# zhangganlin/GlORIE-SLAM

Hardware: AMD Instinct MI355X
Metric: DSPO BA-update iters/sec + rendered rays/sec, 640x480 Replica keyframe graph (higher is better)
Workload: dtype f16 corr/ConvGRU, f32 Jacobians, f64 solve; render: f32 (decoder matmuls as 3-term f16 splits, f32 accumulate); 1 GPU; G8: 8 keyframes, 36 edges, 60x80 (640x480/8), BA itrs=2, DSPO stages alternating, context part of the GRU gates (one map per source keyframe) re-evaluated for all keyframes every 12 steps; multiview_filter.thresh = 0.25 (reference ships 0.01, configs/mono_point_slam.yaml:75: with untrained weights 0.01 rejects > 80 % of every frame and no depth_scale step would reach stage 2); render: 524k-point c; edges_local=36, edges_total=36, hw=4800, keyframes=8, parallelism=single GPU

## Files before the change

### glorie_slam_amd/_lib.py

```python
import ctypes
import os
import threading

import torch

_PKG_DIR = os.path.dirname(os.path.abspath(__file__))
LIB_PATH = os.path.join(_PKG_DIR, "lib", "libglorie_hip.so")

GLORIE_F16, GLORIE_F32 = 0, 1
_STATUS = {0: "GLORIE_OK", -1: "GLORIE_EINVAL", -2: "GLORIE_EHIP", -3: "GLORIE_ENOMEM",
           -4: "GLORIE_EUNSUPPORTED"}

_c_int, _c_f, _vp, _sz = ctypes.c_int, ctypes.c_float, ctypes.c_void_p, ctypes.c_size_t

SIGNATURES = {
    "glorie_version": (ctypes.c_char_p, []),
    "glorie_last_hip_error": (_c_int, []),
    "glorie_ctx_create": (_c_int, [ctypes.POINTER(_vp), _sz]),
    "glorie_ctx_destroy": (_c_int, [_vp]),
    "glorie_ctx_reserve": (_c_int, [_vp, _sz]),
    "glorie_ctx_generation": (ctypes.c_ulonglong, [_vp]),
    "glorie_corr_index_fwd": (_c_int, [_vp, _vp, _vp] + [_c_int] * 7 + [_vp]),
    "glorie_corr_lookup_pyramid": (_c_int, [_vp, _c_int, _vp, _vp] + [_c_int] * 7 + [_vp]),
    "glorie_corr_otf": (_c_int, [_vp, _vp, _c_int, _vp, _vp, _vp, _vp] + [_c_int] * 4 + [_vp]),
    "glorie_corr_otf_encode": (_c_int, [_vp, _vp, _c_int, _vp, _vp, _vp, _vp] + [_c_int] * 4 + [_vp, _vp, _vp, _c_int, _vp]),
    "glorie_altcorr_fwd": (_c_int, [_vp] * 4 + [_c_int] * 8 + [_vp]),
    "glorie_bias_act": (_c_int, [_vp, _c_int, _vp, _vp, _c_int, ctypes.c_long, _c_int, _c_int, _vp]),
    "glorie_gru_glo_terms": (_c_int, [_vp, _c_int, _vp, _vp, _c_int, _vp, _vp, _c_int, _vp, _c_int, _vp, _c_int, _c_int, _vp]),
    "glorie_gru_gate_zr": (_c_int, [_vp, _c_int, _vp, _c_int, _vp, _c_int, _vp, _c_int, _vp, _c_int, _c_int, _c_int, _vp]),
    "glorie_gru_gate_q": (_c_int, [_vp, _c_int, _vp, _c_int, _vp, _c_int, _vp, _c_int, _vp, _c_int, _vp, _c_int, _c_int, _c_int, _vp]),
    "glorie_segment_mean": (_c_int, [_vp, _c_int, _vp, _c_int, _vp, _c_int, _vp, _c_int, _c_int, _c_int, _vp]),
    "glorie_conv3x3_small": (_c_int, [_vp, _c_int, _vp, _c_int, _vp, _vp, _c_int, _c_int, _c_int, ctypes.c_float, _vp, _vp, _c_int, _c_int, _c_int, _vp]),
    "glorie_gru_glo_from_tiles": (_c_int, [_vp, _vp, _vp, _c_int, _vp, _c_int, _c_int, _vp]),
    "glorie_update_bookkeeping": (_c_int, [_vp, _vp, _vp, ctypes.c_long, _vp, _vp, _vp, _vp, _c_int, _c_int, _c_f, _vp, _c_int,
                                           _vp]),
    "glorie_conv_igemm_heads": (_c_int, [_vp, _c_int, _c_int, _vp, _c_int, _c_int, _vp, _vp, _c_int, _c_int, _vp, _vp,
                                         _c_int, _c_int, _c_int, _c_int, _vp]),
    "glorie_conv_upsample": (_c_int, [_vp, _c_int, _c_int, _vp, _vp, _vp, _vp, _vp, _c_int, _c_int, _c_int, _c_int, _vp]),
    "glorie_conv_stencil": (_c_int, [_vp, _vp, _c_int, _c_int, _c_int, ctypes.c_float, _vp, _vp, _c_int, _c_int, _c_int, _vp]),
    "glorie_conv_igemm": (_c_int, [_vp, _c_int, _c_int, _vp, _c_int, _c_int, _vp, _c_int, _c_int, _c_int, _vp,
                                   _c_int, _c_int, _vp, _c_int, _vp, _c_int, _vp, _c_int, _vp, _c_int, _vp, _c_int, _vp,
                                   _c_int, _c_int, _c_int, _vp]),
    "glorie_flow_conv7": (_c_int, [_vp, _vp, _vp, _vp, _c_int, _c_int, _c_int, _c_int, _vp]),
    "glorie_motion": (_c_int, [_vp, _vp, _vp, _vp, _c_int, _c_int, _c_int, ctypes.c_float, _vp]),
    "glorie_motion_padded": (_c_int, [_vp, _vp, _vp, _vp, _c_int, _c_int, _c_int, ctypes.c_float, _vp]),
    "glorie_flow_pad": (_c_int, [_vp, _vp, _c_int, _c_int, _c_int, _vp]),
    "glorie_flow_conv7_padded": (_c_int, [_vp, _vp, _vp, _vp, _c_int, _c_int, _c_int, _c_int, _vp]),
    "glorie_flow_encoder": (_c_int, [_vp, _vp, _vp, _vp, _vp, _vp, _c_int, _c_int, _c_int, _c_int, _vp]),
    "glorie_publish_flag": (_c_int, [_vp, _vp, _vp, _vp]),
    "glorie_dspo_prepare": (_c_int, [_vp] * 4 + [_c_int] * 4 + [ctypes.c_float, _c_int, ctypes.c_float, _vp, _vp, _c_int] + [_vp] * 9),
    "glorie_corr_lookup_pyramid_tiled": (_c_int, [_vp, _c_int, _vp, _vp] + [_c_int] * 5 + [_vp]),
    "glorie_corr_build": (_c_int, [_vp] * 5 + [_c_int] * 5 + [_vp]),
    "glorie_corr_lookup_arena": (_c_int, [_vp, _c_int, _vp, _vp, _vp] + [_c_int] * 5 + [_vp]),
    "glorie_corr_lookup_tiled_cl": (_c_int, [_vp, _c_int, _vp, _vp, _c_int, _vp] + [_c_int] * 5 + [_vp]),
    "glorie_corr_dm_level_halfs": (ctypes.c_long, [_c_int, _c_int, _c_int]),
    "glorie_corr_dm_build": (_c_int, [_vp] * 5 + [_c_int] * 5 + [_vp]),
    "glorie_corr_dm_lookup": (_c_int, [_vp, _vp, _vp, _c_int, _c_int, _c_int, _c_int, _vp, _vp, _vp, _vp, _c_int, _vp]),
    "glorie_valid_depth_mask": (_c_int, [_vp] * 4 + [_c_int] * 4 + [ctypes.c_float, _c_int, _vp, _vp, _vp]),
    "glorie_reproject": (_c_int, [_vp] * 7 + [_c_int] * 3 + [_vp]),
    "glorie_reproject_motion": (_c_int, [_vp] * 9 + [_c_int] * 3 + [ctypes.c_float, _vp]),
    "glorie_frame_distance": (_c_int, [_vp] * 6 + [_c_int] * 3 + [_c_f, _vp]),
    "glorie_iproj": (_c_int, [_vp] * 4 + [_c_int] * 3 + [_vp]),
# ... 221 lines not shown
```

### glorie_slam_amd/csrc/gru.hip

```cpp
#include <hip/hip_runtime.h>
#include <stdint.h>
#include "common.hiph"

namespace glorie {

typedef __attribute__((ext_vector_type(8))) _Float16 h8;

__device__ __forceinline__ float sigmoidf_(float x) { return 1.0f / (1.0f + __expf(-x)); }
__device__ __forceinline__ float tanhf_(float x) {
  const float e = __expf(-2.0f * fabsf(x));
  const float t = (1.0f - e) / (1.0f + e);
  return copysignf(t, x);
}

enum { ACT_NONE = 0, ACT_RELU = 1, ACT_SIGMOID = 2, ACT_SOFTPLUS = 3 };

template <int C8T>
__global__ __launch_bounds__(256) void bias_act_kernel(const _Float16* __restrict__ x, int xs,
                                                       const float* __restrict__ bias,
                                                       _Float16* __restrict__ y, int ys, long P,
                                                       int C8R, int act) {
  const int C8 = C8T ? C8T : C8R;
  const long idx = (long)blockIdx.x * 256 + threadIdx.x;
  if (idx >= P * C8) return;
// ... 109 lines not shown
                                                         const _Float16* __restrict__ net, int ns,
                                                         _Float16* __restrict__ out, int os,
                                                         _Float16* __restrict__ out2, int os2, long P,
                                                         int HW) {
  const long idx = (long)blockIdx.x * 256 + threadIdx.x;
  if (idx >= P * 16) return;
  const long p = idx >> 4;
  const int c = (int)(idx & 15) * 8;
  const int n = (int)(p / HW);
  const h8 qv = *reinterpret_cast<const h8*>(qc + p * qs + c);
  const h8 zv = *reinterpret_cast<const h8*>(z + p * zs + c);
  const h8 nv = *reinterpret_cast<const h8*>(net + p * ns + c);
  h8 o;
#pragma unroll
  for (int k = 0; k < 8; ++k) {
    const float q = tanhf_((float)qv[k] + gq[(size_t)n * gs + c + k]);
    const float zz = (float)zv[k];
    o[k] = (_Float16)((1.0f - zz) * (float)nv[k] + zz * q);
  }
  *reinterpret_cast<h8*>(out + p * os + c) = o;
  if (out2) *reinterpret_cast<h8*>(out2 + p * os2 + c) = o;
}

__global__ __launch_bounds__(256) void segment_mean_kernel(const _Float16* __restrict__ x, int xs,
                                                           const float* __restrict__ bias, int relu,
                                                           const int64_t* __restrict__ ix, int N,
                                                           _Float16* __restrict__ out, int os, int HW) {
  __shared__ int elist[256];
  __shared__ int wcnt[4];
  const int tid = threadIdx.x, lane = tid & 63, wv = tid >> 6;
  const int idx = blockIdx.x * 256 + tid;
  const bool live = idx < HW * 16;
  const int p = idx >> 4, c = (idx & 15) * 8, g = blockIdx.y;
  float b[8] = {0, 0, 0, 0, 0, 0, 0, 0};
  if (bias) {
#pragma unroll
    for (int k = 0; k < 8; ++k) b[k] = bias[c + k];
  }
  float acc[8] = {0, 0, 0, 0, 0, 0, 0, 0};
  int cnt = 0;
  for (int base = 0; base < N; base += 256) {
    const int e = base + tid;
    const bool hit = e < N && ix[e] == g;
    const unsigned long long m = __ballot(hit);
    if (lane == 0) wcnt[wv] = __popcll(m);
    __syncthreads();
    int off = 0, total = 0;
#pragma unroll
    for (int q = 0; q < 4; ++q) {
      if (q < wv) off += wcnt[q];
      total += wcnt[q];
    }
    if (hit) elist[off + __popcll(m & ((1ull << lane) - 1ull))] = e;
    __syncthreads();
    if (live) {
      for (int q = 0; q < total; ++q) {
        const h8 v = *reinterpret_cast<const h8*>(x + ((long)elist[q] * HW + p) * xs + c);
#pragma unroll
        for (int k = 0; k < 8; ++k) {
          float f = (float)v[k] + b[k];
          if (relu) f = fmaxf(f, 0.0f);
          acc[k] += f;
        }
      }
    }
    cnt += total;
    __syncthreads();
  }
  if (!live) return;
  const float inv = 1.0f / (float)max(cnt, 1);
  h8 o;
#pragma unroll
  for (int k = 0; k < 8; ++k) o[k] = (_Float16)(acc[k] * inv);
  *reinterpret_cast<h8*>(out + ((long)g * HW + p) * os + c) = o;
}

typedef __attribute__((ext_vector_type(8))) _Float16 f16x8;
typedef __attribute__((ext_vector_type(4))) float f32x4;

template <int NT>
__global__ __launch_bounds__(256) void conv_taps_kernel(const _Float16* __restrict__ x, int xs,
                                                        const float* __restrict__ in_bias, int in_relu,
                                                        const f16x8* __restrict__ wp,
                                                        float* __restrict__ taps, int ncols, int tstride,
                                                        long P) {
  const int lane = threadIdx.x & 63, wv = threadIdx.x >> 6;
  const int col = lane & 15, kg = lane >> 4;
  const int grp = blockIdx.y;
  f16x8 bfrag[NT][4];
#pragma unroll
  for (int t = 0; t < NT; ++t)
#pragma unroll
    for (int kk = 0; kk < 4; ++kk) bfrag[t][kk] = wp[(((size_t)grp * NT + t) * 4 + kk) * 64 + lane];
  float ib[4][8];
#pragma unroll
  for (int kk = 0; kk < 4; ++kk)
#pragma unroll
// ... 17 lines not shown
        }
    }
#pragma unroll
    for (int t = 0; t < NT; ++t) {
      f32x4 acc = f32x4{0.f, 0.f, 0.f, 0.f};
#pragma unroll
      for (int kk = 0; kk < 4; ++kk)
        acc = __builtin_amdgcn_mfma_f32_16x16x32_f16(afrag[kk], bfrag[t][kk], acc, 0, 0, 0);
      const int n = t * 16 + col;
      if (n < ncols) {
#pragma unroll
        for (int r = 0; r < 4; ++r) {
          const long pr = p0 + kg * 4 + r;
          if (pr < P) taps[pr * tstride + grp * ncols + n] = acc[r];
        }
      }
    }
  }
}

__device__ __forceinline__ float softplusf_(float x) { return x > 20.0f ? x : log1pf(__expf(x)); }

template <bool PLANAR>
__global__ __launch_bounds__(256) void conv_stencil_kernel(const float* __restrict__ taps, int ncols,
                                                           int tstride, const float* __restrict__ bias,
                                                           int K, int groups, int act_packed, float scale,
                                                           float* __restrict__ out, long P, int H, int W,
                                                           float* __restrict__ out_last = nullptr) {
  const long idx = (long)blockIdx.x * 256 + threadIdx.x;
  if (idx >= P * K * groups) return;
  const int gk = PLANAR ? (int)(idx / P) : (int)(idx % (K * groups));
  const long p = PLANAR ? idx - (long)gk * P : idx / (K * groups);
  const int grp = gk / K, j = gk - grp * K;
  const int xw = (int)(p % W), yh = (int)((p / W) % H);
  float acc = bias ? bias[grp * K + j] : 0.0f;
#pragma unroll
  for (int d = 0; d < 9; ++d) {
    const int dy = d / 3 - 1, dx = d % 3 - 1;
    if ((unsigned)(yh + dy) < (unsigned)H && (unsigned)(xw + dx) < (unsigned)W)
      acc += PLANAR ? taps[(size_t)(grp * ncols + d * K + j) * P + (p + dy * W + dx)]
                    : taps[(p + dy * W + dx) * tstride + grp * ncols + d * K + j];
  }
  const int act = (act_packed >> (4 * grp)) & 15;
  if (act == ACT_RELU) acc = fmaxf(acc, 0.0f);
  else if (act == ACT_SIGMOID) acc = sigmoidf_(acc);
  else if (act == ACT_SOFTPLUS) acc = softplusf_(acc);
  if (out_last && grp == groups - 1) out_last[(size_t)p * K + j] = acc * scale;
  else out[((size_t)grp * P + p) * K + j] = acc * scale;
}

}

using namespace glorie;

extern "C" int glorie_bias_act(const void* x, int x_stride, const float* bias, void* y, int y_stride,
                               long P, int C, int act, void* stream) {
  if (P < 0 || C <= 0 || (C & 7) || (x_stride & 7) || (y_stride & 7)) return GLORIE_EINVAL;
  if (P == 0) return GLORIE_OK;
  if (!x || !y) return GLORIE_EINVAL;
  const long total = P * (C / 8);
  const dim3 grid((unsigned)((total + 255) / 256));
  auto launch = [&](auto kernel) {
    hipLaunchKernelGGL(kernel, grid, dim3(256), 0, (hipStream_t)stream,
                       reinterpret_cast<const _Float16*>(x), x_stride, bias,
                       reinterpret_cast<_Float16*>(y), y_stride, P, C / 8, act);
  };
  switch (C / 8) {
    case 8: launch(bias_act_kernel<8>); break;
    case 16: launch(bias_act_kernel<16>); break;
    case 48: launch(bias_act_kernel<48>); break;
    default: launch(bias_act_kernel<0>); break;
// ... 165 lines not shown
    hipLaunchKernelGGL(conv_taps_kernel<1>, dim3(gx, groups), dim3(256), 0, st,
                       reinterpret_cast<const _Float16*>(x), x_stride, in_bias, in_relu,
                       reinterpret_cast<const f16x8*>(w_packed), taps, ncols, tstride, P);
  else
    hipLaunchKernelGGL(conv_taps_kernel<2>, dim3(gx, groups), dim3(256), 0, st,
                       reinterpret_cast<const _Float16*>(x), x_stride, in_bias, in_relu,
                       reinterpret_cast<const f16x8*>(w_packed), taps, ncols, tstride, P);
  const long total = P * K * groups;
  hipLaunchKernelGGL(conv_stencil_kernel<false>, dim3((unsigned)((total + 255) / 256)), dim3(256), 0, st, taps,
                     ncols, tstride, out_bias, K, groups, act_packed, scale, out, P, H, W);
  return check_launch();
}

extern "C" int glorie_conv_stencil(const float* taps, const float* out_bias, int groups, int K, int act_packed,
                                   float scale, float* out, float* out_last, int N, int H, int W, void* stream) {
  if (N < 0 || H <= 0 || W <= 0 || groups < 1 || groups > 4 || K < 1 || K > 3) return GLORIE_EINVAL;
  if (N == 0) return GLORIE_OK;
  if (!taps || !out) return GLORIE_EINVAL;
  const long P = (long)N * H * W, total = P * K * groups;
  hipLaunchKernelGGL(conv_stencil_kernel<true>, dim3((unsigned)((total + 255) / 256)), dim3(256), 0, (hipStream_t)stream,
                     taps, 9 * K, 9 * K * groups, out_bias, K, groups, act_packed, scale, out, P, H, W, out_last);
  return check_launch();
}
```

### glorie_slam_amd/droid_net.py

```python
import os

import numpy as np
import torch
import torch.nn as nn
import torch.nn.functional as F

from . import droid_backends


def _conv(cin, cout, k):
    return nn.Conv2d(cin, cout, kernel_size=(k, k), padding=(k // 2, k // 2))


def cvx_upsample(data, mask):
    batch, ht, wd, dim = data.shape
    mask = mask.reshape(batch, 576, ht, wd)
    ix = torch.arange(batch, device=data.device)
    out = torch.empty(batch, 8 * ht, 8 * wd, dim, dtype=torch.float32, device=data.device)
    for c in range(dim):
        up = torch.empty(batch, 8 * ht, 8 * wd, dtype=torch.float32, device=data.device)
        droid_backends.cvx_upsample(data[..., c].float().contiguous(), ix, mask.contiguous(), up, softmax_f32=True)
        out[..., c] = up
    return out

# ... 193 lines not shown
    def __call__(self, net, inp, corr, flow=None, ii=None, jj=None, groups=None):
        self._sync()
        return self._net(self._cl(net), self._cl(inp), self._cl(corr), self._cl(flow), ii, jj, groups)


class FusedUpdate:

    def __init__(self, module, inplace=False):
        self.src = module
        self.inplace = inplace
        self.hoist_inp = True
        self._pre = None
        self.parallel = False
        self.glo_stream = True
        self._streams = None
        self._ver = None
        self._hx = None
        self._inp_key = None
        self._pre_kf, self._pre_map, self._ctx_key = None, None, None
        self._flow_pad = None
        self.fuse_glo = True
        self.fuse_heads = True
        self.fuse_flow = os.environ.get("GLORIE_FLOW_FUSED", "1") != "0"
        self.gate_events = None
        self.q_events = None
        self.heads_events = None
        self.corr_events = None

    def _sync(self):
        from . import update_ops as U
        ver = tuple(p._version for p in self.src.parameters())
        if self._ver == ver:
            return
        m = self.src
        f32 = lambda b: b.detach().float().contiguous()
        g = m.gru
        W = {}
        W["ce1_t"] = m.corr_encoder[0].weight.detach().view(128, -1).t().half().contiguous()
        W["ce1_b"] = f32(m.corr_encoder[0].bias)
        W["ce1_p"] = OtfCorrBlock.pack_encoder(m.corr_encoder[0].weight)
        W["ce1_cl"] = U.pack_corr_encoder(m.corr_encoder[0].weight)
        W["ce1_dm"] = U.pack_corr_encoder_dm(m.corr_encoder[0].weight)
        W["ce2"], W["ce2_b"] = U.pack_conv_igemm(m.corr_encoder[2].weight, pair=True), f32(m.corr_encoder[2].bias)
        W["fe1"], W["fe1_b"] = U.pack_flow_conv7(m.flow_encoder[0].weight), f32(m.flow_encoder[0].bias)
        W["fe2"], W["fe2_b"] = U.pack_conv_igemm(m.flow_encoder[2].weight, pair=True), f32(m.flow_encoder[2].bias)
        W["zr"] = U.pack_conv_igemm(torch.cat([g.convz.weight, g.convr.weight], 0), pair=True)
# ... 18 lines not shown
        W["up"], W["up_b"] = U.pack_conv_igemm(m.agg.upmask[0].weight), f32(m.agg.upmask[0].bias)
        W["up_cvx"], W["up_cvx_b"] = U.pack_upmask_conv(m.agg.upmask[0].weight, m.agg.upmask[0].bias)
        self.W = W
        self._ver = ver
        self._inp_key = None

    @torch.no_grad()
    def precompute_context(self):
        from . import update_ops as U
        hx = self._hx
        n, _, ht, wd = hx.shape
        if self._pre is None or self._pre.shape[0] != n or self._pre.shape[2:] != hx.shape[2:] \
                or self._pre.device != hx.device:
            self._pre = torch.empty((n, 384, ht, wd), dtype=torch.float16, device=hx.device,
                                    memory_format=torch.channels_last)
        U.conv_igemm(hx[:, 0:128], None, self.W["pre"], 9, 384, self._pre)
        return self._pre

    @staticmethod
    def _cl(t):
        b, n, c, h, w = t.shape
        return t.reshape(b * n, c, h, w).half().contiguous(memory_format=torch.channels_last)

    def _side_streams(self, dev):
        if self._streams is None or self._streams[0].device != dev:
            self._streams = (torch.cuda.Stream(dev), torch.cuda.Stream(dev))
        return self._streams

    @torch.no_grad()
    def precompute_shared_context(self, context):
        from . import update_ops as U
        table, frames, index = context
        g = int(frames.shape[0])
        ht, wd = table.shape[-2:]
        x = table[frames].half().contiguous(memory_format=torch.channels_last)
        if self._pre_kf is None or self._pre_kf.shape[0] < g or tuple(self._pre_kf.shape[2:]) != (ht, wd) \
                or self._pre_kf.device != x.device:
            self._pre_kf = torch.empty((max(g, 8), 384, ht, wd), dtype=torch.float16, device=x.device,
                                       memory_format=torch.channels_last)
        U.conv_igemm(x, None, self.W["pre"], 9, 384, self._pre_kf[:g])
        n = int(index.shape[0])
        if self._pre_map is None or self._pre_map.shape[0] < n or self._pre_map.device != x.device:
            self._pre_map = torch.zeros(max(n, 64), dtype=torch.int32, device=x.device)
        self._pre_map[:n].copy_(index)
        return self._pre_kf[:g], self._pre_map[:n]

    def _shared_context(self, context):
        table, frames, index = context
        key = (table.data_ptr(), table._version, frames.data_ptr(), frames._version, index.data_ptr(), index._version,
               int(frames.shape[0]), int(index.shape[0]), self._ver)
        if self._ctx_key != key:
            self.precompute_shared_context(context)
            self._ctx_key = key
            self._ctx_refs = (table, frames, index)
        return self._pre_kf[:int(frames.shape[0])], self._pre_map[:int(index.shape[0])]

    @torch.no_grad()
    def __call__(self, net, inp, corr, flow=None, ii=None, jj=None, groups=None, context=None, lazy_up=False,
                 weight_out=None):
        from . import update_ops as U
        self._sync()
        W = self.W
        batch, num, _, ht, wd = net.shape
        n, hw = batch * num, ht * wd
        dev = net.device
        cl_map = lambda c: torch.empty((n, c, ht, wd), dtype=torch.float16, device=dev,
                                       memory_format=torch.channels_last)
        if self._hx is None or tuple(self._hx.shape) != (n, 320, ht, wd) or self._hx.device != dev:
            self._hx = cl_map(320)
            self._inp_key = None
        hx = self._hx
        net0 = self._cl(net)
        main = torch.cuda.current_stream(dev)
        side = self._side_streams(dev) if self.parallel else ((main, self._side_streams(dev)[1]) if self.glo_stream
                                                              else (main, main))
        for st in side:
            if st is not main:
                st.wait_stream(main)
        with torch.cuda.stream(side[0]):
            if isinstance(flow, U.PaddedFlow):
                pf = flow
            else:
# ... 1 lines not shown
                    flow = torch.zeros(batch, num, 4, ht, wd, device=dev)
                fl = flow.reshape(n, 4, ht, wd).permute(0, 2, 3, 1).float().contiguous()
                if self._flow_pad is None or not self._flow_pad.fits(n, ht, wd, dev):
                    self._flow_pad = U.PaddedFlow(n, ht, wd, dev)
                pf = U.flow_pad(fl, self._flow_pad)
            if not (self.fuse_flow and U.flow_encoder(pf, W["fe1"], W["fe1_b"], W["fe2"], W["fe2_b"], hx[:, 256:320],
                                                      strict=False)):
                f1 = U.flow_conv7_padded(pf, W["fe1"], W["fe1_b"], cl_map(128))
                U.conv_igemm(f1, None, W["fe2"], 9, 64, hx[:, 256:320], terms=W["fe2_b"], act=U.ACT_RELU)
        shared = context is not None and self.hoist_inp
        with torch.cuda.stream(side[1]):
            if shared:
                pre_kf, pre_map = self._shared_context(context)
            elif self._inp_key is None or self._inp_key[0] is not inp or self._inp_key[1] != inp._version:
                U.bias_act(self._cl(inp), None, U.ACT_NONE, out=hx[:, 0:128])
                self._inp_key = (inp, inp._version)
                if self.hoist_inp:
                    self.precompute_context()
            if self.fuse_glo:
                g = U.gru_glo_terms_fused(net0, W["w"], W["w_b"], W["G"], W["G_b"])
            else:
                wn = U.conv_igemm(net0, None, W["w"], 1, 128, cl_map(128))
                g = U.gru_glo_terms(wn, W["w_b"], net0, W["G"], W["G_b"])
        if self.glo_stream and not self.parallel:
            main.wait_stream(side[1])
        if hasattr(corr, "encode_into"):
            c1 = cl_map(128)
            evc = self.corr_events
            if evc is not None:
                c0e, c1e = torch.cuda.Event(enable_timing=True), torch.cuda.Event(enable_timing=True)
                c0e.record()
            corr.encode_into(W, c1)
            if evc is not None:
                c1e.record()
                evc.append((c0e, c1e))
        else:
            if callable(corr):
                corr = corr()
            if corr.dim() == 4 and corr.shape[1] == 256 and corr.dtype == torch.float16:
                c1 = U.conv_igemm(corr, None, W["ce1_cl"], 1, 128, cl_map(128), terms=W["ce1_b"], act=U.ACT_RELU)
            else:
                c1 = torch.matmul(corr.reshape(n, -1, hw).half().transpose(1, 2), W["ce1_t"])
                c1 = c1.view(n, ht, wd, 128).permute(0, 3, 1, 2)
                U.bias_act(c1, W["ce1_b"], U.ACT_RELU)
        U.conv_igemm(c1, None, W["ce2"], 9, 128, hx[:, 128:256], terms=W["ce2_b"], act=U.ACT_RELU)
        for st in side:
            if st is not main:
                main.wait_stream(st)
        z, rnet = cl_map(128), cl_map(128)
        aliased = net0.data_ptr() == net.data_ptr() and net.dtype == torch.float16
        new = net0 if (self.inplace and aliased) else cl_map(128)
        if self.hoist_inp:
            dynx = hx[:, 128:320]
            pre, pmap = (pre_kf, pre_map) if shared else (self._pre, None)
            ev = self.gate_events
            if ev is not None:
                e0, e1 = torch.cuda.Event(enable_timing=True), torch.cuda.Event(enable_timing=True)
                e0.record()
            U.conv_igemm(net0, dynx, W["zr_dyn"], 9, 256, z, epilogue=U.EPI_GRU_ZR, terms=g[:, 0:256], net=net0,
                         out2=rnet, pre=pre[:, 0:256], pre_map=pmap)
            if ev is not None:
                e1.record()
                ev.append((e0, e1))
            evq = self.q_events
            if evq is not None:
                q0, q1 = torch.cuda.Event(enable_timing=True), torch.cuda.Event(enable_timing=True)
                q0.record()
            U.conv_igemm(rnet, dynx, W["q_dyn"], 9, 128, new, epilogue=U.EPI_GRU_Q, terms=g[:, 256:384], net=net0,
                         z=z, pre=pre[:, 256:384], pre_map=pmap)
            if evq is not None:
                q1.record()
                evq.append((q0, q1))
        else:
            U.conv_igemm(net0, hx, W["zr"], 9, 256, z, epilogue=U.EPI_GRU_ZR, terms=g[:, 0:256], net=net0, out2=rnet)
            U.conv_igemm(rnet, hx, W["q"], 9, 128, new, epilogue=U.EPI_GRU_Q, terms=g[:, 256:384], net=net0, z=z)
        net_out = new.view(batch, num, 128, ht, wd)
        if self.fuse_heads:
            agg_in = cl_map(128)
            evh = self.heads_events
            if evh is not None:
                h0, h1e = torch.cuda.Event(enable_timing=True), torch.cuda.Event(enable_timing=True)
                h0.record()
            rows = U.conv_igemm_heads(new, W["h1"], 9, 384, W["h1_b"], W["h2_taps"], 2, out=agg_in)
            if evh is not None:
                h1e.record()
                evh.append((h0, h1e))
            wo = weight_out if (weight_out is not None and weight_out.is_cuda and weight_out.dtype == torch.float32
                                and weight_out.is_contiguous() and weight_out.numel() == n * ht * wd * 2) else None
            dw = U.conv_stencil(rows, W["h2_b"], n, ht, wd, 2, 2, (U.ACT_NONE, U.ACT_SIGMOID), out_last=wo)
        else:
            h1 = U.conv_igemm(new, None, W["h1"], 9, 384, cl_map(384), terms=W["h1_b"], act=U.ACT_RELU)
            dw = U.conv3x3_small(h1, W["h2"], W["h2_b"], 2, (U.ACT_NONE, U.ACT_SIGMOID))
            agg_in = h1[:, 256:384]
        delta = dw[0].view(batch, num, ht, wd, 2)
        weight = dw[1].view(batch, num, ht, wd, 2) if (not self.fuse_heads or wo is None) else \
            weight_out.view(batch, num, ht, wd, 2)
        if ii is None:
            return net_out, delta, weight
        if groups is None:
            uniq, ix = torch.unique(ii.to(dev), sorted=True, return_inverse=True)
            ngroups = uniq.shape[0]
        else:
            ix, ngroups = groups
        agg = U.segment_mean(agg_in, ix.contiguous(), ngroups)
        a2 = torch.empty((ngroups, 128, ht, wd), dtype=torch.float16, device=dev,
                         memory_format=torch.channels_last)
        U.conv_igemm(agg, None, W["a2"], 9, 128, a2, terms=W["a2_b"], act=U.ACT_RELU)
        eta = U.conv3x3_small(a2, W["eta"], W["eta_b"], 1, (U.ACT_SOFTPLUS,), scale=0.01)
        if lazy_up:
            return net_out, delta, weight, eta.view(batch, ngroups, ht, wd), U.LazyUpmask(a2, W["up_cvx"], W["up_cvx_b"])
        up = torch.empty((ngroups, 576, ht, wd), dtype=torch.float16, device=dev,
                         memory_format=torch.channels_last)
        U.conv_igemm(a2, None, W["up"], 1, 576, up, terms=W["up_b"])
        return net_out, delta, weight, eta.view(batch, ngroups, ht, wd), up.view(batch, ngroups, 576, ht, wd)


class CorrBlock:

    def __init__(self, fmap1, fmap2, num_levels=4, radius=3, tiled=None):
        self.num_levels = num_levels
        self.radius = radius
        corr = CorrBlock.corr(fmap1, fmap2)
        batch, num, h1, w1, h2, w2 = corr.shape
        self.dims = (h1, w1, h2, w2)
        if tiled is None:
            tiled = corr.is_cuda and radius == 3 and (h1 * w1) % 8 == 0 and corr.dtype == torch.float16
        self.tiled = bool(tiled)
        corr = corr.reshape(batch * num * h1 * w1, 1, h2, w2)
        self.corr_pyramid = []
        for i in range(num_levels):
            if self.tiled:
# ... 298 lines not shown
```

### glorie_slam_amd/factor_graph.py

```python
import numpy as np
import os

import torch

from . import droid_backends
from .droid_net import ArenaLookup, CorrArena, CorrBlock, AltCorrBlock, FusedUpdate, FusedLookup, OtfCorrBlock


def coords_grid(ht, wd, device):
    y, x = torch.meshgrid(torch.arange(ht, device=device).float(),
                          torch.arange(wd, device=device).float(), indexing="ij")
    return torch.stack([x, y], dim=-1)


class FactorGraph:
    def __init__(self, video, update_op, device="cuda:0", corr_impl="volume", max_factors=-1,
                 use_graphs=False, capture_after=1):
        self.video = video
        self.update_op = update_op
        self.device = device
        self.max_factors = max_factors
        self.corr_impl = corr_impl
        self.ht = ht = video.ht // video.down_scale
        self.wd = wd = video.wd // video.down_scale
# ... 317 lines not shown
                and self.target.dtype == torch.float32:
            pf = self._padded_flow(int(self.ii.shape[0]), self.target.device)
            coords1, mask = self.video.reproject(self.ii, self.jj, motion=(self.target, pf))
            motn = pf
        else:
            coords1, mask = self.video.reproject(self.ii, self.jj)
            motn = self._motion(coords1, padded=self.fast_update is not None)
        if self.corr_impl == "otf":
            blk = self._otf_block()
            rig = self._otf_rig
            ck = ("otf_idx", rig)
            if ck not in self._graphs:
                self._graphs[ck] = ((rig * self.ii).contiguous(), (rig * self.jj + (self.ii == self.jj).long()).contiguous())
            oi, oj = self._graphs[ck]
            lookup = FusedLookup(blk, coords1, oi, oj) if (self.fast_update is not None and blk.num_levels == 4) \
                else (lambda: blk(coords1, oi, oj))
        elif self.fast_update is not None and isinstance(self.corr, CorrArena) and self.corr.layout == "dm":
            lookup = ArenaLookup(self.corr, coords1)
        elif self.fast_update is not None and isinstance(self.corr, (CorrArena, CorrBlock)):
            lookup = lambda: self.corr(coords1, channels_last=True)
        else:
            lookup = lambda: self.corr(coords1)
        uniq = self._unique_ii()
        if self.fast_update is not None:
            ix, _ = self._groups()
            self.net, delta, weight, damping, upmask = \
                self.fast_update(self.net, self.inp, lookup, motn, self.ii, self.jj, self._groups(),
                                 context=(self.video.inps, uniq, ix) if self.share_context else None,
                                 lazy_up=True, weight_out=self.weight)
        else:
            corr = lookup()
            with torch.autocast("cuda", enabled=True):
                self.net, delta, weight, damping, upmask = \
                    self.update_op(self.net, self.inp, corr, motn, self.ii, self.jj)
        if t0 is None or t1 is None:
            t0, t1 = self._window(t0, t1, use_inactive)
        sharded = self.video.is_sharded()
        fused_book = (self.fast_update is not None and not use_inactive and not sharded and coords1.is_cuda
                      and self.target.shape == coords1.shape and self.target.dtype == torch.float32
                      and self.target.is_contiguous() and coords1.is_contiguous() and coords1.dtype == torch.float32
                      and delta.dtype == torch.float32 and delta.is_contiguous() and delta.shape == coords1.shape
                      and damping.dtype == torch.float32 and damping.is_contiguous()
                      and self.damping.dtype == torch.float32 and self.damping.is_contiguous()
                      and damping.numel() == uniq.shape[0] * self.ht * self.wd and self.age.is_contiguous())
        damping_ba = None
        if fused_book:
            from . import _lib as L
            damping_ba = torch.empty((uniq.shape[0], self.ht, self.wd), dtype=torch.float32, device=coords1.device)
            L.check(L.load().glorie_update_bookkeeping(
                L.ptr(coords1), L.ptr(delta), L.ptr(self.target), coords1.numel(), L.ptr(damping), L.ptr(uniq),
                L.ptr(self.damping), L.ptr(damping_ba), int(uniq.shape[0]), self.ht * self.wd, float(EP), L.ptr(self.age),
                int(self.age.shape[0]), L.stream_ptr()), "glorie_update_bookkeeping")
            self._age_done = True
        elif self.target.shape == coords1.shape and self.target.dtype == torch.float32 and self.target.is_contiguous():
            torch.add(coords1, delta.to(dtype=torch.float), out=self.target)
        else:
            self.target = coords1 + delta.to(dtype=torch.float)
        self.weight = weight.to(dtype=torch.float)
        if not fused_book:
            self.damping[uniq] = damping.to(self.damping.dtype)
        if use_inactive:
            ck = ("inac", t0)
            c = self._graphs.get(ck)
            if c is None:
                m = (self.ii_inac >= t0 - 3) & (self.jj_inac >= t0 - 3)
                ii_c = torch.cat([self.ii_inac[m], self.ii], 0)
                jj_c = torch.cat([self.jj_inac[m], self.jj], 0)
                tgt = torch.cat([self.target_inac[:, m], self.target], 1)
                wgt = torch.cat([self.weight_inac[:, m], self.weight], 1)
# ... 213 lines not shown
```

### glorie_slam_amd/update_ops.py

```python
import torch

from . import _lib as L

ACT_NONE, ACT_RELU, ACT_SIGMOID, ACT_SOFTPLUS = 0, 1, 2, 3


def _rows(t, name):
    if t.dtype != torch.float16 or t.dim() != 4:
        raise RuntimeError(f"{name}: expected a 4-D float16 map, got {t.dtype} {tuple(t.shape)}")
    n, c, h, w = t.shape
    sn, sc, sh, sw = t.stride()
    if c > 1 and sc != 1:
        raise RuntimeError(f"{name}: not channels-last (channel stride {sc})")
    if (w > 1 and sh != w * sw) or (h * w > 1 and n > 1 and sn != h * w * sw) or sw < c:
        raise RuntimeError(f"{name}: rows are not uniformly strided {tuple(t.stride())}")
    if sw % 8 or t.data_ptr() % 16:
        raise RuntimeError(f"{name}: rows must be 16-byte aligned")
    return sw


def bias_act(x, bias, act, out=None):
    L.need_cuda(x)
    out = x if out is None else out
    xs, ys = _rows(x, "x"), _rows(out, "out")
# ... 237 lines not shown
                                             L.ptr(tap_w), groups, K, L.ptr(rows), L.ptr(out) if rest else None,
                                             _rows(out, "out") if rest else 0, n, h, w, L.stream_ptr()),
            "glorie_conv_igemm_heads")
    return rows


def conv_stencil(rows, out_bias, n, h, w, groups, K, acts, scale=1.0, out_last=None):
    L.need_cuda(rows)
    if rows.dtype != torch.float32 or tuple(rows.shape) != (groups * 9 * K, n * h * w) or not rows.is_contiguous() \
            or len(acts) != groups:
        raise RuntimeError("conv_stencil: bad tap planes")
    out = torch.empty((groups, n, h, w, K), dtype=torch.float32, device=rows.device)
    packed = 0
    for gidx, a in enumerate(acts):
        packed |= int(a) << (4 * gidx)
    if out_last is not None and (out_last.dtype != torch.float32 or not out_last.is_contiguous() or not out_last.is_cuda
                                 or out_last.numel() != n * h * w * K):
        raise RuntimeError("conv_stencil: out_last must be a contiguous float32 CUDA tensor of n*h*w*K elements")
    L.check(L.load().glorie_conv_stencil(L.ptr(rows), L.ptr(out_bias), groups, K, packed, float(scale), L.ptr(out),
                                         L.ptr(out_last), n, h, w, L.stream_ptr()), "glorie_conv_stencil")
    return out


def pack_flow_conv7(weight):
    if tuple(weight.shape) != (128, 4, 7, 7):
        raise RuntimeError("pack_flow_conv7: expected [128,4,7,7]")
    w = torch.zeros(128, 7, 8, 4, dtype=torch.float16, device=weight.device)
    w[:, :, :7] = weight.detach().permute(0, 2, 3, 1).half()
    return w.reshape(128, 224).contiguous()


def pack_upmask_conv(weight, bias):
    if weight.shape[0] != 576 or tuple(weight.shape[2:]) != (1, 1):
        raise RuntimeError("pack_upmask_conv: expected a [576, C, 1, 1] weight")
    C = weight.shape[1]
    w = weight.detach().reshape(9, 8, 8, C)
    wp = torch.zeros(8, 8, 16, C, dtype=w.dtype, device=w.device)
    wp[:, :, :9] = w.permute(1, 2, 0, 3)
    bp = torch.zeros(8, 8, 16, dtype=torch.float32, device=w.device)
    bp[:, :, :9] = bias.detach().float().reshape(9, 8, 8).permute(1, 2, 0)
    return pack_conv_igemm(wp.reshape(1024, C, 1, 1)), bp.reshape(1024).contiguous()


class LazyUpmask:

    def __init__(self, x, w_packed, bias):
# ... 91 lines not shown
```

### include/glorie_hip.h

```cpp
#ifndef GLORIE_HIP_H
#define GLORIE_HIP_H

#include <stdint.h>
#include <stddef.h>

#ifdef __cplusplus
extern "C" {
#endif

typedef enum glorie_status {
  GLORIE_OK = 0,
  GLORIE_EINVAL = -1,
  GLORIE_EHIP = -2,
  GLORIE_ENOMEM = -3,
  GLORIE_EUNSUPPORTED = -4
} glorie_status;

typedef enum glorie_dtype { GLORIE_F16 = 0, GLORIE_F32 = 1 } glorie_dtype;

const char* glorie_version(void);
int glorie_last_hip_error(void);

typedef struct glorie_ctx glorie_ctx;

// ... 63 lines not shown
                      int o2_stride, int N, int HW, void* stream);
int glorie_segment_mean(const void* x, int x_stride, const float* bias, int relu, const int64_t* ix,
                        int N, void* out, int o_stride, int G, int HW, void* stream);
int glorie_conv3x3_small(const void* x, int x_stride, const float* in_bias, int in_relu,
                         const void* w_packed, const float* out_bias, int groups, int K,
                         int act_packed, float scale, float* taps, float* out, int N, int H, int W,
                         void* stream);

#define GLORIE_CONV_PAIR16 0x100
int glorie_conv_igemm(const void* xa, int xa_stride, int ca, const void* xb, int xb_stride, int cb,
                      const void* w_packed, int taps, int nout, int epilogue, const float* terms,
                      int terms_stride, int act, const void* net, int net_stride, const void* z,
                      int z_stride, void* out, int out_stride, void* out2, int out2_stride,
                      const void* pre, int pre_stride, const int* pre_map, int N, int H, int W, void* stream);

int glorie_conv_igemm_heads(const void* x, int x_stride, int c, const void* w_packed, int taps, int nout,
                            const float* bias, const void* tap_w, int groups, int K, float* tap_out, void* out,
                            int out_stride, int N, int H, int W, void* stream);
int glorie_conv_upsample(const void* x, int x_stride, int c, const void* w_packed, const float* bias,
                         const float* disps, const int64_t* ix, float* disps_up, int softmax_f32, int M, int H, int W,
                         void* stream);
int glorie_conv_stencil(const float* taps, const float* out_bias, int groups, int K, int act_packed, float scale,
                        float* out, float* out_last, int N, int H, int W, void* stream);

int glorie_flow_conv7(const float* flow, const void* w_packed, const float* bias, void* out,
                      int out_stride, int N, int H, int W, void* stream);

int glorie_flow_pad(const float* flow, void* padded, int N, int H, int W, void* stream);
int glorie_flow_conv7_padded(const void* padded, const void* w_packed, const float* bias, void* out, int out_stride,
                             int N, int H, int W, void* stream);

int glorie_flow_encoder(const void* padded, const void* w7_packed, const float* b7, const void* w3_packed, const float* b3,
                        void* out, int out_stride, int N, int H, int W, void* stream);


int glorie_reproject(const float* poses, const float* disps, const float* intrinsics,
                     const int64_t* ii, const int64_t* jj, float* coords, float* valid,
                     int N, int h, int w, void* stream);

int glorie_frame_distance(const float* poses, const float* disps, const float* intrinsics,
                          const int64_t* ii, const int64_t* jj, float* dist,
                          int K, int h, int w, float beta, void* stream);

int glorie_iproj(const float* poses, const float* disps, const float* intrinsics,
                 float* points, int num, int h, int w, void* stream);

// ... 313 lines not shown
```

Baseline: 968.4 BA-update iters/s.

## Fuse update-operator tail: heads stencil with segment mean, eta conv with bookkeeping

Adds a heads_finish kernel that runs the delta/weight stencil and the per-keyframe segment-mean aggregation in a single launch, and also writes target = coords1 + delta. Adds an eta_finish kernel that does the eta 3x3 conv through MFMA into LDS, applies softplus, and writes eta, the damping table, damping_ba and the age increment, replacing the separate bookkeeping launch. The goal is fewer kernel launches and fewer intermediate round trips per update iteration. The cost is a more complex gated path and tighter coupling between the factor graph and the operator. It also drops a redundant wait on the glo stream.

After: 984.8 BA-update iters/s, median of 6. 1.02x the previous value.

```diff
diff --git a/glorie_slam_amd/_lib.py b/glorie_slam_amd/_lib.py
--- a/glorie_slam_amd/_lib.py
+++ b/glorie_slam_amd/_lib.py
@@ -38,6 +38,10 @@
                                          _c_int, _c_int, _c_int, _c_int, _vp]),
     "glorie_conv_upsample": (_c_int, [_vp, _c_int, _c_int, _vp, _vp, _vp, _vp, _vp, _c_int, _c_int, _c_int, _c_int, _vp]),
     "glorie_conv_stencil": (_c_int, [_vp, _vp, _c_int, _c_int, _c_int, ctypes.c_float, _vp, _vp, _c_int, _c_int, _c_int, _vp]),
+    "glorie_heads_finish": (_c_int, [_vp, _vp, _c_int, _c_int, _c_int, _c_f, _vp, _vp, _vp, _vp, _vp, _c_int, _vp, _c_int, _vp,
+                                     _vp, _c_int, _c_int, _c_int, _c_int, _c_int, _vp]),
+    "glorie_eta_finish": (_c_int, [_vp, _c_int, _vp, _vp, _c_f, _vp, _vp, _vp, _vp, _c_f, _vp, _c_int, _c_int, _c_int, _c_int,
+                                   _c_int, _vp]),
     "glorie_conv_igemm": (_c_int, [_vp, _c_int, _c_int, _vp, _c_int, _c_int, _vp, _c_int, _c_int, _c_int, _vp,
                                    _c_int, _c_int, _vp, _c_int, _vp, _c_int, _vp, _c_int, _vp, _c_int, _vp, _c_int, _vp,
                                    _c_int, _c_int, _c_int, _vp]),
diff --git a/glorie_slam_amd/csrc/gru.hip b/glorie_slam_amd/csrc/gru.hip
--- a/glorie_slam_amd/csrc/gru.hip
+++ b/glorie_slam_amd/csrc/gru.hip
@@ -155,16 +155,16 @@
   if (out2) *reinterpret_cast<h8*>(out2 + p * os2 + c) = o;
 }
 
-__global__ __launch_bounds__(256) void segment_mean_kernel(const _Float16* __restrict__ x, int xs,
-                                                           const float* __restrict__ bias, int relu,
-                                                           const int64_t* __restrict__ ix, int N,
-                                                           _Float16* __restrict__ out, int os, int HW) {
+__device__ __forceinline__ void segment_mean_body(int bx, int g, const _Float16* __restrict__ x, int xs,
+                                                  const float* __restrict__ bias, int relu,
+                                                  const int64_t* __restrict__ ix, int N,
+                                                  _Float16* __restrict__ out, int os, int HW) {
   __shared__ int elist[256];
   __shared__ int wcnt[4];
   const int tid = threadIdx.x, lane = tid & 63, wv = tid >> 6;
-  const int idx = blockIdx.x * 256 + tid;
+  const int idx = bx * 256 + tid;
   const bool live = idx < HW * 16;
-  const int p = idx >> 4, c = (idx & 15) * 8, g = blockIdx.y;
+  const int p = idx >> 4, c = (idx & 15) * 8;
   float b[8] = {0, 0, 0, 0, 0, 0, 0, 0};
   if (bias) {
 #pragma unroll
@@ -206,6 +206,13 @@
 #pragma unroll
   for (int k = 0; k < 8; ++k) o[k] = (_Float16)(acc[k] * inv);
   *reinterpret_cast<h8*>(out + ((long)g * HW + p) * os + c) = o;
+}
+
+__global__ __launch_bounds__(256) void segment_mean_kernel(const _Float16* __restrict__ x, int xs,
+                                                           const float* __restrict__ bias, int relu,
+                                                           const int64_t* __restrict__ ix, int N,
+                                                           _Float16* __restrict__ out, int os, int HW) {
+  segment_mean_body(blockIdx.x, blockIdx.y, x, xs, bias, relu, ix, N, out, os, HW);
 }
 
 typedef __attribute__((ext_vector_type(8))) _Float16 f16x8;
@@ -269,12 +276,12 @@
 __device__ __forceinline__ float softplusf_(float x) { return x > 20.0f ? x : log1pf(__expf(x)); }
 
 template <bool PLANAR>
-__global__ __launch_bounds__(256) void conv_stencil_kernel(const float* __restrict__ taps, int ncols,
-                                                           int tstride, const float* __restrict__ bias,
-                                                           int K, int groups, int act_packed, float scale,
-                                                           float* __restrict__ out, long P, int H, int W,
-                                                           float* __restrict__ out_last = nullptr) {
-  const long idx = (long)blockIdx.x * 256 + threadIdx.x;
+__device__ __forceinline__ void conv_stencil_body(long idx, const float* __restrict__ taps, int ncols,
+                                                  int tstride, const float* __restrict__ bias,
+                                                  int K, int groups, int act_packed, float scale,
+                                                  float* __restrict__ out, long P, int H, int W,
+                                                  float* __restrict__ out_last, const float* __restrict__ coords1,
+                                                  float* __restrict__ target) {
   if (idx >= P * K * groups) return;
   const int gk = PLANAR ? (int)(idx / P) : (int)(idx % (K * groups));
   const long p = PLANAR ? idx - (long)gk * P : idx / (K * groups);
@@ -292,8 +299,105 @@
   if (act == ACT_RELU) acc = fmaxf(acc, 0.0f);
   else if (act == ACT_SIGMOID) acc = sigmoidf_(acc);
   else if (act == ACT_SOFTPLUS) acc = softplusf_(acc);
-  if (out_last && grp == groups - 1) out_last[(size_t)p * K + j] = acc * scale;
-  else out[((size_t)grp * P + p) * K + j] = acc * scale;
+  const float v = acc * scale;
+  if (out_last && grp == groups - 1) out_last[(size_t)p * K + j] = v;
+  else out[((size_t)grp * P + p) * K + j] = v;
+  if (target && grp == 0) {
+#pragma clang fp contract(off)
+    target[(size_t)p * K + j] = coords1[(size_t)p * K + j] + v;
+  }
+}
+
+template <bool PLANAR>
+__global__ __launch_bounds__(256) void conv_stencil_kernel(const float* __restrict__ taps, int ncols,
+                                                           int tstride, const float* __restrict__ bias,
+                                                           int K, int groups, int act_packed, float scale,
+                                                           float* __restrict__ out, long P, int H, int W,
+                                                           float* __restrict__ out_last = nullptr) {
+  conv_stencil_body<PLANAR>((long)blockIdx.x * 256 + threadIdx.x, taps, ncols, tstride, bias, K, groups, act_packed, scale,
+                            out, P, H, W, out_last, nullptr, nullptr);
+}
+
+__global__ __launch_bounds__(256) void heads_finish_kernel(const float* __restrict__ taps, int ncols, int tstride,
+                                                           const float* __restrict__ bias, int K, int groups,
+                                                           int act_packed, float scale, float* __restrict__ out, long P,
+                                                           int H, int W, float* __restrict__ out_last,
+                                                           const float* __restrict__ coords1, float* __restrict__ target,
+                                                           unsigned nb_stencil, const _Float16* __restrict__ x, int xs,
+                                                           const float* __restrict__ mbias, int relu,
+                                                           const int64_t* __restrict__ ix, int N,
+                                                           _Float16* __restrict__ agg, int os, int nbx) {
+  if (blockIdx.x < nb_stencil) {
+    conv_stencil_body<true>((long)blockIdx.x * 256 + threadIdx.x, taps, ncols, tstride, bias, K, groups, act_packed, scale,
+                            out, P, H, W, out_last, coords1, target);
+  } else {
+    const int b = (int)(blockIdx.x - nb_stencil);
+    segment_mean_body(b % nbx, b / nbx, x, xs, mbias, relu, ix, N, agg, os, H * W);
+  }
+}
+
+__global__ __launch_bounds__(256) void eta_finish_kernel(const _Float16* __restrict__ x, int xs,
+                                                         const f16x8* __restrict__ wp, const float* __restrict__ bias,
+                                                         float scale, float* __restrict__ eta,
+                                                         const int64_t* __restrict__ frames,
+                                                         float* __restrict__ damping_table,
+                                                         float* __restrict__ damping_ba, float ep,
+                                                         int64_t* __restrict__ age, int n_edges, int G, int H, int W,
+                                                         int R, int nrb) {
+  extern __shared__ float tapl[];
+  const int tid = threadIdx.x, lane = tid & 63, wv = tid >> 6;
+  if (age)
+    for (long i = (long)blockIdx.x * 256 + tid; i < n_edges; i += (long)gridDim.x * 256) age[i] += 1;
+  if (blockIdx.x >= (unsigned)(G * nrb)) return;
+  const int g = blockIdx.x / nrb, r0 = (blockIdx.x - g * nrb) * R;
+  const int r1 = min(r0 + R, H), ra = max(r0 - 1, 0), rb = min(r1 + 1, H);
+  const int npx = (rb - ra) * W;
+  const long HW = (long)H * W, base = (long)g * HW + (long)ra * W;
+  const int col = lane & 15, kg = lane >> 4;
+  f16x8 bfrag[4];
+#pragma unroll
+  for (int kk = 0; kk < 4; ++kk) bfrag[kk] = wp[kk * 64 + lane];
+  const int ntiles = (npx + 15) / 16;
+  for (int tile = wv; tile < ntiles; tile += 4) {
+    const int p0 = tile * 16;
+    const int pa = min(p0 + col, npx - 1);
+    const f16x8* src = reinterpret_cast<const f16x8*>(x + (base + pa) * xs + kg * 8);
+    f16x8 afrag[4];
+#pragma unroll
+    for (int kk = 0; kk < 4; ++kk) afrag[kk] = src[kk * 4];
+    f32x4 acc = f32x4{0.f, 0.f, 0.f, 0.f};
+#pragma unroll
+    for (int kk = 0; kk < 4; ++kk) acc = __builtin_amdgcn_mfma_f32_16x16x32_f16(afrag[kk], bfrag[kk], acc, 0, 0, 0);
+    if (col < 9) {
+#pragma unroll
+      for (int r = 0; r < 4; ++r) {
+        const int pr = p0 + kg * 4 + r;
+        if (pr < npx) tapl[pr * 9 + col] = acc[r];
+      }
+    }
+  }
+  __syncthreads();
+  const int nown = (r1 - r0) * W;
+  for (int q = tid; q < nown; q += 256) {
+    const int yl = q / W, xw = q - yl * W, yh = r0 + yl;
+    float acc = bias ? bias[0] : 0.0f;
+#pragma unroll
+    for (int d = 0; d < 9; ++d) {
+      const int dy = d / 3 - 1, dx = d % 3 - 1;
+      if ((unsigned)(yh + dy) < (unsigned)H && (unsigned)(xw + dx) < (unsigned)W)
+        acc += tapl[((yh + dy - ra) * W + xw + dx) * 9 + d];
+    }
+    acc = softplusf_(acc);
+    const float e = acc * scale;
+    const long qm = (long)yh * W + xw, i = (long)g * HW + qm;
+    eta[i] = e;
+    {
+#pragma clang fp contract(off)
+      damping_table[(size_t)frames[g] * HW + qm] = e;
+      const float m = e * 0.2f;
+      damping_ba[i] = m + ep;
+    }
+  }
 }
 
 }
@@ -505,3 +609,44 @@
                      taps, 9 * K, 9 * K * groups, out_bias, K, groups, act_packed, scale, out, P, H, W, out_last);
   return check_launch();
 }
+
+extern "C" int glorie_heads_finish(const float* taps, const float* out_bias, int groups, int K, int act_packed, float scale,
+                                   float* out, float* out_last, const float* coords1, float* target, const void* x,
+                                   int x_stride, const float* bias, int relu, const int64_t* ix, void* agg, int o_stride,
+                                   int G, int N, int H, int W, void* stream) {
+  if (N < 0 || G < 0 || H <= 0 || W <= 0 || groups < 1 || groups > 4 || K < 1 || K > 3 || (x_stride & 7) || (o_stride & 7) ||
+      (coords1 == nullptr) != (target == nullptr))
+    return GLORIE_EINVAL;
+  if (N == 0 && G == 0) return GLORIE_OK;
+  if ((N > 0 && (!taps || !out)) || (G > 0 && (!agg || (N > 0 && (!x || !ix))))) return GLORIE_EINVAL;
+  const long HW = (long)H * W, P = (long)N * HW, total = P * K * groups;
+  const long nb_stencil = (total + 255) / 256, nbx = (HW * 16 + 255) / 256;
+  if (HW * 16 > 0x7fffffffL || nb_stencil + nbx * G > 0x7fffffffL) return GLORIE_EINVAL;
+  hipLaunchKernelGGL(heads_finish_kernel, dim3((unsigned)(nb_stencil + nbx * G)), dim3(256), 0, (hipStream_t)stream, taps,
+                     9 * K, 9 * K * groups, out_bias, K, groups, act_packed, scale, out, P, H, W, out_last, coords1, target,
+                     (unsigned)nb_stencil, reinterpret_cast<const _Float16*>(x), x_stride, bias, relu, ix, N,
+                     reinterpret_cast<_Float16*>(agg), o_stride, (int)nbx);
+  return check_launch();
+}
+
+extern "C" int glorie_eta_finish(const void* x, int x_stride, const void* w_packed, const float* out_bias, float scale,
+                                 float* eta, const int64_t* frames, float* damping_table, float* damping_ba, float ep,
+                                 int64_t* age, int n_edges, int rows_per_block, int G, int H, int W, void* stream) {
+  if (G < 0 || H <= 0 || W <= 0 || n_edges < 0 || rows_per_block < 0 || (x_stride & 7)) return GLORIE_EINVAL;
+  const int n_age = age ? n_edges : 0;
+  if (G == 0 && n_age == 0) return GLORIE_OK;
+  if (G > 0 && (!x || !w_packed || !eta || !frames || !damping_table || !damping_ba)) return GLORIE_EINVAL;
+  const long lds_row = (long)W * 9 * sizeof(float), lds_max = 64 * 1024;
+  int R = rows_per_block ? rows_per_block : 2;
+  if (R > H) R = H;
+  if (!rows_per_block && min(R + 2, H) * lds_row > lds_max) R = 1;
+  const int lds_rows = min(R + 2, H);
+  if (lds_rows * lds_row > lds_max) return GLORIE_EUNSUPPORTED;
+  const int nrb = (H + R - 1) / R;
+  const long nb = max((long)G * nrb, 1L);
+  if (nb > 0x7fffffffL) return GLORIE_EINVAL;
+  hipLaunchKernelGGL(eta_finish_kernel, dim3((unsigned)nb), dim3(256), (size_t)(lds_rows * lds_row), (hipStream_t)stream,
+                     reinterpret_cast<const _Float16*>(x), x_stride, reinterpret_cast<const f16x8*>(w_packed), out_bias,
+                     scale, eta, frames, damping_table, damping_ba, ep, age, n_age, G, H, W, R, nrb);
+  return check_launch();
+}
diff --git a/glorie_slam_amd/droid_net.py b/glorie_slam_amd/droid_net.py
--- a/glorie_slam_amd/droid_net.py
+++ b/glorie_slam_amd/droid_net.py
@@ -239,6 +239,7 @@
         self.fuse_glo = True
         self.fuse_heads = True
         self.fuse_flow = os.environ.get("GLORIE_FLOW_FUSED", "1") != "0"
+        self.fuse_tail = os.environ.get("GLORIE_TAIL_FUSED", "1") != "0"
         self.gate_events = None
         self.q_events = None
         self.heads_events = None
@@ -303,6 +304,14 @@
         b, n, c, h, w = t.shape
         return t.reshape(b * n, c, h, w).half().contiguous(memory_format=torch.channels_last)
 
+    @staticmethod
+    def _agg_groups(ii, groups, dev):
+        if groups is None:
+            uniq, ix = torch.unique(ii.to(dev), sorted=True, return_inverse=True)
+            return ix.contiguous(), uniq.shape[0]
+        ix, ngroups = groups
+        return ix.contiguous(), ngroups
+
     def _side_streams(self, dev):
         if self._streams is None or self._streams[0].device != dev:
             self._streams = (torch.cuda.Stream(dev), torch.cuda.Stream(dev))
@@ -338,7 +347,7 @@
 
     @torch.no_grad()
     def __call__(self, net, inp, corr, flow=None, ii=None, jj=None, groups=None, context=None, lazy_up=False,
-                 weight_out=None):
+                 weight_out=None, book=None):
         from . import update_ops as U
         self._sync()
         W = self.W
@@ -386,8 +395,10 @@
             else:
                 wn = U.conv_igemm(net0, None, W["w"], 1, 128, cl_map(128))
                 g = U.gru_glo_terms(wn, W["w_b"], net0, W["G"], W["G_b"])
+        joined = None
         if self.glo_stream and not self.parallel:
             main.wait_stream(side[1])
+            joined = side[1]
         if hasattr(corr, "encode_into"):
             c1 = cl_map(128)
             evc = self.corr_events
@@ -409,7 +420,7 @@
                 U.bias_act(c1, W["ce1_b"], U.ACT_RELU)
         U.conv_igemm(c1, None, W["ce2"], 9, 128, hx[:, 128:256], terms=W["ce2_b"], act=U.ACT_RELU)
         for st in side:
-            if st is not main:
+            if st is not main and st is not joined:
                 main.wait_stream(st)
         z, rnet = cl_map(128), cl_map(128)
         aliased = net0.data_ptr() == net.data_ptr() and net.dtype == torch.float16
@@ -439,6 +450,7 @@
             U.conv_igemm(net0, hx, W["zr"], 9, 256, z, epilogue=U.EPI_GRU_ZR, terms=g[:, 0:256], net=net0, out2=rnet)
             U.conv_igemm(rnet, hx, W["q"], 9, 128, new, epilogue=U.EPI_GRU_Q, terms=g[:, 256:384], net=net0, z=z)
         net_out = new.view(batch, num, 128, ht, wd)
+        tail = book is not None and self.fuse_tail and self.fuse_heads and ii is not None
         if self.fuse_heads:
             agg_in = cl_map(128)
             evh = self.heads_events
@@ -451,7 +463,12 @@
                 evh.append((h0, h1e))
             wo = weight_out if (weight_out is not None and weight_out.is_cuda and weight_out.dtype == torch.float32
                                 and weight_out.is_contiguous() and weight_out.numel() == n * ht * wd * 2) else None
-            dw = U.conv_stencil(rows, W["h2_b"], n, ht, wd, 2, 2, (U.ACT_NONE, U.ACT_SIGMOID), out_last=wo)
+            if tail:
+                ix, ngroups = self._agg_groups(ii, groups, dev)
+                dw, agg = U.heads_finish(rows, W["h2_b"], n, ht, wd, 2, 2, (U.ACT_NONE, U.ACT_SIGMOID), agg_in, ix, ngroups,
+                                         out_last=wo, coords1=book.coords1, target=book.target)
+            else:
+                dw = U.conv_stencil(rows, W["h2_b"], n, ht, wd, 2, 2, (U.ACT_NONE, U.ACT_SIGMOID), out_last=wo)
         else:
             h1 = U.conv_igemm(new, None, W["h1"], 9, 384, cl_map(384), terms=W["h1_b"], act=U.ACT_RELU)
             dw = U.conv3x3_small(h1, W["h2"], W["h2_b"], 2, (U.ACT_NONE, U.ACT_SIGMOID))
@@ -461,16 +478,26 @@
             weight_out.view(batch, num, ht, wd, 2)
         if ii is None:
             return net_out, delta, weight
-        if groups is None:
-            uniq, ix = torch.unique(ii.to(dev), sorted=True, return_inverse=True)
-            ngroups = uniq.shape[0]
-        else:
-            ix, ngroups = groups
-        agg = U.segment_mean(agg_in, ix.contiguous(), ngroups)
+        if not tail:
+            ix, ngroups = self._agg_groups(ii, groups, dev)
+            agg = U.segment_mean(agg_in, ix, ngroups)
         a2 = torch.empty((ngroups, 128, ht, wd), dtype=torch.float16, device=dev,
                          memory_format=torch.channels_last)
         U.conv_igemm(agg, None, W["a2"], 9, 128, a2, terms=W["a2_b"], act=U.ACT_RELU)
-        eta = U.conv3x3_small(a2, W["eta"], W["eta_b"], 1, (U.ACT_SOFTPLUS,), scale=0.01)
+        eta = None
+        if tail:
+            eta = U.eta_finish(a2, W["eta"], W["eta_b"], book.frames, book.damping_table, book.damping_ba, book.ep, book.age,
+                               scale=0.01, strict=False)
+        if eta is None:
+            eta = U.conv3x3_small(a2, W["eta"], W["eta_b"], 1, (U.ACT_SOFTPLUS,), scale=0.01)
+            if tail:
+                L = U.L
+                L.check(L.load().glorie_update_bookkeeping(
+                    None, None, None, 0, L.ptr(eta), L.ptr(book.frames), L.ptr(book.damping_table), L.ptr(book.damping_ba),
+                    ngroups, hw, book.ep, L.ptr(book.age), int(book.age.numel()) if book.age is not None else 0,
+                    L.stream_ptr()), "glorie_update_bookkeeping")
+        if tail:
+            book.done = True
         if lazy_up:
             return net_out, delta, weight, eta.view(batch, ngroups, ht, wd), U.LazyUpmask(a2, W["up_cvx"], W["up_cvx_b"])
         up = torch.empty((ngroups, 576, ht, wd), dtype=torch.float16, device=dev,
diff --git a/glorie_slam_amd/factor_graph.py b/glorie_slam_amd/factor_graph.py
--- a/glorie_slam_amd/factor_graph.py
+++ b/glorie_slam_amd/factor_graph.py
@@ -363,12 +363,22 @@
         else:
             lookup = lambda: self.corr(coords1)
         uniq = self._unique_ii()
+        book = None
         if self.fast_update is not None:
             ix, _ = self._groups()
+            if (getattr(self.fast_update, "fuse_tail", False) and self.fast_update.fuse_heads and not use_inactive
+                    and not self.video.is_sharded() and coords1.is_cuda
+                    and self.target.shape == coords1.shape and self.target.dtype == torch.float32
+                    and self.target.is_contiguous() and coords1.is_contiguous() and coords1.dtype == torch.float32
+                    and self.damping.dtype == torch.float32 and self.damping.is_contiguous() and self.age.is_contiguous()):
+                from .update_ops import TailBook
+                book = TailBook(coords1, self.target, uniq, self.damping,
+                                torch.empty((uniq.shape[0], self.ht, self.wd), dtype=torch.float32, device=coords1.device),
+                                EP, self.age)
             self.net, delta, weight, damping, upmask = \
                 self.fast_update(self.net, self.inp, lookup, motn, self.ii, self.jj, self._groups(),
                                  context=(self.video.inps, uniq, ix) if self.share_context else None,
-                                 lazy_up=True, weight_out=self.weight)
+                                 lazy_up=True, weight_out=self.weight, book=book)
         else:
             corr = lookup()
             with torch.autocast("cuda", enabled=True):
@@ -385,7 +395,11 @@
                       and self.damping.dtype == torch.float32 and self.damping.is_contiguous()
                       and damping.numel() == uniq.shape[0] * self.ht * self.wd and self.age.is_contiguous())
         damping_ba = None
-        if fused_book:
+        if book is not None and book.done:
+            assert fused_book, "the operator did the bookkeeping on tensors the bookkeeping launch would not take"
+            damping_ba = book.damping_ba
+            self._age_done = True
+        elif fused_book:
             from . import _lib as L
             damping_ba = torch.empty((uniq.shape[0], self.ht, self.wd), dtype=torch.float32, device=coords1.device)
             L.check(L.load().glorie_update_bookkeeping(
diff --git a/glorie_slam_amd/update_ops.py b/glorie_slam_amd/update_ops.py
--- a/glorie_slam_amd/update_ops.py
+++ b/glorie_slam_amd/update_ops.py
@@ -283,6 +283,73 @@
     return out
 
 
+class TailBook:
+
+    def __init__(self, coords1, target, frames, damping_table, damping_ba, ep, age):
+        self.coords1, self.target, self.frames, self.damping_table = coords1, target, frames, damping_table
+        self.damping_ba, self.ep, self.age = damping_ba, float(ep), age
+        self.done = False
+
+
+def _f32c(t, numel, name):
+    if not t.is_cuda or t.dtype != torch.float32 or not t.is_contiguous() or t.numel() != numel:
+        raise RuntimeError(f"{name} must be a contiguous float32 CUDA tensor of {numel} elements")
+
+
+def heads_finish(rows, out_bias, n, h, w, groups, K, acts, x, ix, ngroups, scale=1.0, out_last=None, coords1=None,
+                 target=None):
+    L.need_cuda(rows, x, ix)
+    if rows.dtype != torch.float32 or tuple(rows.shape) != (groups * 9 * K, n * h * w) or not rows.is_contiguous() \
+            or len(acts) != groups:
+        raise RuntimeError("heads_finish: bad tap planes")
+    if tuple(x.shape) != (n, 128, h, w) or ix.dtype != torch.int64 or ix.numel() != n or not ix.is_contiguous():
+        raise RuntimeError("heads_finish: x must be [N,128,h,w], ix int64 [N]")
+    if out_last is not None:
+        _f32c(out_last, n * h * w * K, "heads_finish: out_last")
+    if (coords1 is None) != (target is None):
+        raise RuntimeError("heads_finish: coords1 and target come together")
+    if coords1 is not None:
+        _f32c(coords1, n * h * w * K, "heads_finish: coords1")
+        _f32c(target, n * h * w * K, "heads_finish: target")
+    out = torch.empty((groups, n, h, w, K), dtype=torch.float32, device=rows.device)
+    agg = torch.empty((ngroups, 128, h, w), dtype=torch.float16, device=x.device, memory_format=torch.channels_last)
+    packed = 0
+    for gidx, a in enumerate(acts):
+        packed |= int(a) << (4 * gidx)
+    L.check(L.load().glorie_heads_finish(L.ptr(rows), L.ptr(out_bias), groups, K, packed, float(scale), L.ptr(out),
+                                         L.ptr(out_last), L.ptr(coords1), L.ptr(target), L.ptr(x), _rows(x, "x"), None, 0,
+                                         L.ptr(ix), L.ptr(agg), 128, ngroups, n, h, w, L.stream_ptr()),
+            "glorie_heads_finish")
+    return out, agg
+
+
+def eta_finish(x, w_packed, out_bias, frames, damping_table, damping_ba, ep, age=None, scale=1.0, rows_per_block=0,
+               strict=True):
+    L.need_cuda(x, w_packed, frames, damping_table, damping_ba, age)
+    g, c, h, w = x.shape
+    if c != 128 or w_packed.dtype != torch.float16 or tuple(w_packed.shape) != (1, 1, 4, 64, 8) or not w_packed.is_contiguous():
+        raise RuntimeError("eta_finish: x must be [G,128,h,w], w_packed = pack_conv3x3_small of one [1,128,3,3] weight")
+    if frames.dtype != torch.int64 or frames.numel() != g or not frames.is_contiguous():
+        raise RuntimeError("eta_finish: frames must be a contiguous int64 [G]")
+    if damping_table.dtype != torch.float32 or not damping_table.is_contiguous() or damping_table.dim() < 2 \
+            or damping_table[0].numel() != h * w:
+        raise RuntimeError("eta_finish: damping_table must be contiguous float32 [B,h,w]")
+    _f32c(damping_ba, g * h * w, "eta_finish: damping_ba")
+    if age is not None and (age.dtype != torch.int64 or not age.is_contiguous()):
+        raise RuntimeError("eta_finish: age must be a contiguous int64 tensor")
+    if out_bias is not None and (out_bias.dtype != torch.float32 or out_bias.numel() != 1):
+        raise RuntimeError("eta_finish: out_bias must be float32 [1]")
+    eta = torch.empty((1, g, h, w, 1), dtype=torch.float32, device=x.device)
+    status = L.load().glorie_eta_finish(L.ptr(x), _rows(x, "x"), L.ptr(w_packed), L.ptr(out_bias), float(scale), L.ptr(eta),
+                                        L.ptr(frames), L.ptr(damping_table), L.ptr(damping_ba), float(ep), L.ptr(age),
+                                        int(age.numel()) if age is not None else 0, int(rows_per_block), g, h, w,
+                                        L.stream_ptr())
+    if status == -4 and not strict:
+        return None
+    L.check(status, "glorie_eta_finish")
+    return eta
+
+
 def pack_flow_conv7(weight):
     if tuple(weight.shape) != (128, 4, 7, 7):
         raise RuntimeError("pack_flow_conv7: expected [128,4,7,7]")
diff --git a/include/glorie_hip.h b/include/glorie_hip.h
--- a/include/glorie_hip.h
+++ b/include/glorie_hip.h
@@ -109,6 +109,13 @@
                          void* stream);
 int glorie_conv_stencil(const float* taps, const float* out_bias, int groups, int K, int act_packed, float scale,
                         float* out, float* out_last, int N, int H, int W, void* stream);
+int glorie_heads_finish(const float* taps, const float* out_bias, int groups, int K, int act_packed, float scale,
+                        float* out, float* out_last, const float* coords1, float* target, const void* x, int x_stride,
+                        const float* bias, int relu, const int64_t* ix, void* agg, int o_stride, int G, int N, int H, int W,
+                        void* stream);
+int glorie_eta_finish(const void* x, int x_stride, const void* w_packed, const float* out_bias, float scale, float* eta,
+                      const int64_t* frames, float* damping_table, float* damping_ba, float ep, int64_t* age, int n_edges,
+                      int rows_per_block, int G, int H, int W, void* stream);
 
 int glorie_flow_conv7(const float* flow, const void* w_packed, const float* bias, void* out,
                       int out_stride, int N, int H, int W, void* stream);
```
